# swyoon/Diffusion-by-MaxEntIRL

Hardware: AMD Instinct MI355X
Metric: images/sec (CIFAR-10 DDPM T=10 generation) (higher is better)
Workload: dtype bf16; 1 GPU; CIFAR-10 DDPM U-Net (35.7M params) VARSampler T=10 generation, 256 images/GPU/step, 3x32x32 (BASELINE configs[1]); noise drawn inside the step; global_batch=256, T=10, parallelism=dp1 (independent trajectories, no collective)

## Files before the change

### diffusion-by-maxentirl_amd/csrc/conv_common.h

```cpp
#pragma once
#include "common.h"

struct ConvArgs {
    const bf16* in0;
    const bf16* in1;
    const bf16* w;
    const float* bias;
    const float* addvec;
    const bf16* residual;
    const bf16* mask_src;
    void* out;
    int N, IH, IW, C0, C1, OH, OW, Cout;
    int ksize, stride, pad, ups, act, addvec_ld, in_mode, out_mode;
    int P, pre_act;
    int TWl, THl, SUBS;
    int HH, HWd;
    int PT, CT, CB, KST;
    int tile_px;
    int lds_buf;
    float mask_slope;
    int stagger;
    int RP, SP;
    float* gn_stats;
    bf16* gn_out;
    const float* gn_gamma;
    const float* gn_beta;
    float gn_eps;
    int gn_flags;
    int res_is_mask;
    int xcd_order;
};

__device__ __forceinline__ int dxmi_xcd_logical(int b, int G, int on) {
    if (!on) return b;
    const int x = b & 7, k = b >> 3;
    const int q = G >> 3, r = G & 7;
    return x * q + (x < r ? x : r) + k;
}

__device__ __forceinline__ float dxmi_row16_sum(float t) {
#define DXMI_DPP_ADD(ctrl) t += __builtin_bit_cast(float, __builtin_amdgcn_update_dpp(0, __builtin_bit_cast(int, t), ctrl, 0xf, 0xf, false))
    DXMI_DPP_ADD(0xB1);
    DXMI_DPP_ADD(0x4E);
    DXMI_DPP_ADD(0x141);
    DXMI_DPP_ADD(0x140);
#undef DXMI_DPP_ADD
    return t;
}

__device__ __forceinline__ void dxmi_stats4(const bf16x4& o, float (&st)[4]) {
    const bf16x2 lo = {o[0], o[1]}, hi = {o[2], o[3]};
    const bf16x2 one = {(bf16)1.f, (bf16)1.f};
    st[0] = __builtin_amdgcn_fdot2_f32_bf16(lo, one, st[0], false);
    st[1] = __builtin_amdgcn_fdot2_f32_bf16(lo, lo, st[1], false);
    st[2] = __builtin_amdgcn_fdot2_f32_bf16(hi, one, st[2], false);
    st[3] = __builtin_amdgcn_fdot2_f32_bf16(hi, hi, st[3], false);
}

__device__ __forceinline__ bool conv_block_to_tile(const ConvArgs& p, int bid, int& pt, int& cot) {
    const int xcd = bid & 7;
    const int j = bid >> 3;
    pt = (j / p.CT) * 8 + xcd;
    cot = j % p.CT;
    return pt < p.PT;
}

template <int MB, int NB, bool WIDE>
__device__ __forceinline__ void conv_epilogue(const ConvArgs& p, f32x16 (&acc)[MB][NB], int pt, int n0, int oy0,
                                              int ox0, int pxblk0, int cb0, int lane) {
    const bool rows = p.in_mode == DXMI_IN_ROWS_F32;
    const int TW = 1 << p.TWl, TH = 1 << p.THl;
    const int h = lane >> 5;
    const bool vec_ok = WIDE || ((p.out_mode != DXMI_OUT_NCHW_F32) && ((p.Cout & 3) == 0));
#pragma unroll
    for (int nb = 0; nb < NB; ++nb) {
        const int pix = (pxblk0 + nb) * 32 + (lane & 31);
        size_t opix;
        int n = 0, oy = 0, ox = 0;
        bool pvalid;
        if (rows) {
            const long grow = (long)pt * p.tile_px + pix;
            pvalid = grow < p.P;
            opix = (size_t)grow;
        } else {
            const int x = pix & (TW - 1);
            const int y = (pix >> p.TWl) & (TH - 1);
            const int sub = pix >> (p.TWl + p.THl);
            n = n0 + sub; oy = oy0 + y; ox = ox0 + x;
            pvalid = n < p.N;
            opix = ((size_t)n * p.OH + oy) * p.OW + ox;
        }
#pragma unroll
        for (int mb = 0; mb < MB; ++mb) {
#pragma unroll
            for (int g = 0; g < 4; ++g) {
                const int co = (cb0 + mb) * 32 + 8 * g + 4 * h;
                float v[4];
#pragma unroll
                for (int e = 0; e < 4; ++e) v[e] = acc[mb][nb][4 * g + e];
                if (pvalid && co < p.Cout) {
                    if (vec_ok) {
                        if (p.bias) {
                            const f32x4 bv = *reinterpret_cast<const f32x4*>(p.bias + co);
#pragma unroll
                            for (int e = 0; e < 4; ++e) v[e] += bv[e];
                        }
                        if (p.addvec) {
                            const f32x4 av = *reinterpret_cast<const f32x4*>(p.addvec + (size_t)n * p.addvec_ld + co);
#pragma unroll
                            for (int e = 0; e < 4; ++e) v[e] += av[e];
                        }
                        if (p.residual) {
                            const bf16x4 rv = *reinterpret_cast<const bf16x4*>(p.residual + opix * p.Cout + co);
#pragma unroll
                            for (int e = 0; e < 4; ++e) v[e] += (float)rv[e];
                        }
                        if (p.mask_src) {
                            const bf16x4 mv = *reinterpret_cast<const bf16x4*>(p.mask_src + opix * p.Cout + co);
#pragma unroll
                            for (int e = 0; e < 4; ++e) v[e] *= ((float)mv[e] > 0.f ? 1.f : p.mask_slope);
                        }
#pragma unroll
                        for (int e = 0; e < 4; ++e) v[e] = dxmi_act(v[e], p.act);
                        if (p.out_mode == DXMI_OUT_ROWS_F32) {
                            f32x4 o;
#pragma unroll
                            for (int e = 0; e < 4; ++e) o[e] = v[e];
                            *reinterpret_cast<f32x4*>(reinterpret_cast<float*>(p.out) + opix * p.Cout + co) = o;
                        } else {
                            bf16x4 o;
#pragma unroll
                            for (int e = 0; e < 4; ++e) o[e] = (bf16)v[e];
                            *reinterpret_cast<bf16x4*>(reinterpret_cast<bf16*>(p.out) + opix * p.Cout + co) = o;
                        }
                    } else if constexpr (!WIDE) {
#pragma unroll
                        for (int e = 0; e < 4; ++e) {
                            if (co + e < p.Cout) {
                                float r = v[e] + (p.bias ? p.bias[co + e] : 0.f);
                                if (p.addvec) r += p.addvec[(size_t)n * p.addvec_ld + co + e];
                                r = dxmi_act(r, p.act);
                                if (p.out_mode == DXMI_OUT_NCHW_F32)
                                    reinterpret_cast<float*>(p.out)[(((size_t)n * p.Cout + co + e) * p.OH + oy) * p.OW + ox] = r;
                                else if (p.out_mode == DXMI_OUT_ROWS_F32)
                                    reinterpret_cast<float*>(p.out)[opix * p.Cout + co + e] = r;
                                else
                                    reinterpret_cast<bf16*>(p.out)[opix * p.Cout + co + e] = (bf16)r;
                            }
                        }
                    }
                }
            }
        }
    }
}

enum class ConvKernel { igemm, pipe, stream1x1, stem, ws, ws8, sm, rw, rw8, head };

struct ConvPlan {
    ConvKernel kind;
    int t0, t1, t2;
    ConvArgs args;
    int grid;
    size_t lds;
    int id;
    int stats_tile;
    bool gn_out;
};

bool conv_ws_select(const ConvArgs& a, ConvPlan* p);
bool conv_ws8_select(const ConvArgs& a, ConvPlan* p);
bool conv_sm_select(const ConvArgs& a, ConvPlan* p);
bool conv1x1_rw_select(const ConvArgs& a, ConvPlan* p);
bool conv1x1_rw8_select(const ConvArgs& a, ConvPlan* p);
bool conv_head_select(const ConvArgs& a, ConvPlan* p);
bool conv_stem_select(const ConvArgs& a, ConvPlan* p);
bool conv_pipe_select(const ConvArgs& a, ConvPlan* p);
int conv_ws_launch(const ConvPlan& p, hipStream_t st);
int conv_ws8_launch(const ConvPlan& p, hipStream_t st);
int conv_sm_launch(const ConvPlan& p, hipStream_t st);
int conv1x1_rw_launch(const ConvPlan& p, hipStream_t st);
int conv1x1_rw8_launch(const ConvPlan& p, hipStream_t st);
int conv_head_launch(const ConvPlan& p, hipStream_t st);
int conv_stem_launch(const ConvPlan& p, hipStream_t st);
int conv_pipe_launch(const ConvPlan& p, hipStream_t st);

template <typename T>
bool conv_zero_page(const void*& page, const T& symbol) {
    void* zp = nullptr;
    if (!page && hipGetSymbolAddress(&zp, symbol) == hipSuccess) page = zp;
    return page != nullptr;
}

int conv_plan(const dxmi_conv_desc* d, ConvPlan* p);
```

### diffusion-by-maxentirl_amd/csrc/conv_ws.hip

```cpp
#include "conv_common.h"
#include <stdlib.h>
#include <type_traits>


#ifdef DXMI_CONV_STAMPS
__device__ unsigned g_ws_wait[256][176];
extern "C" int dxmi_debug_read_ws_stamps(void* dst, int bytes) {
    return (int)hipMemcpyFromSymbol(dst, HIP_SYMBOL(g_ws_wait), bytes, 0, hipMemcpyDeviceToHost);
}
#define WS_STAMPED_BARRIER(idx)                                                                     \
    do {                                                                                            \
        const unsigned long long t0_ = __builtin_amdgcn_s_memtime();                                \
        ws_barrier();                                                                               \
        const unsigned long long t1_ = __builtin_amdgcn_s_memtime();                                \
        if (wave == 0 && lane == 0 && (idx) < 160 && blockIdx.x < 256) g_ws_wait[blockIdx.x][(idx)] = (unsigned)(t1_ - t0_); \
    } while (0)
#define WS_CLOCKSTAMP(slot, cond)                                                                    \
    do {                                                                                            \
        if ((cond) && lane == 0 && blockIdx.x < 256) {                                              \
            g_ws_wait[blockIdx.x][(slot)] = (unsigned)__builtin_amdgcn_s_memtime();                 \
            g_ws_wait[blockIdx.x][(slot) + 1] = (unsigned)__builtin_amdgcn_s_memrealtime();         \
        }                                                                                           \
    } while (0)
#define WS_TSTAMP(slot, cond)                                                                        \
    do {                                                                                            \
        if ((cond) && lane == 0 && blockIdx.x < 256) g_ws_wait[blockIdx.x][(slot)] = (unsigned)__builtin_amdgcn_s_memtime(); \
    } while (0)
#define WS_DBG(bit) (p.stagger & (bit))
#else
#define WS_STAMPED_BARRIER(idx) ws_barrier()
#define WS_TSTAMP(slot, cond) do {} while (0)
#define WS_CLOCKSTAMP(slot, cond) do {} while (0)
#define WS_DBG(bit) 0
#endif

__device__ unsigned long long g_ws_clock[4];
extern "C" int dxmi_conv_ws_last_clock(unsigned long long* host_out4) {
    return hipMemcpyFromSymbol(host_out4, HIP_SYMBOL(g_ws_clock), 4 * sizeof(unsigned long long), 0, hipMemcpyDeviceToHost) == hipSuccess ? DXMI_OK
                                                                                                                                          : DXMI_ELAUNCH;
}

namespace {

constexpr int WS_A_SLOT = 8192;
constexpr int WS_RING = 6;
constexpr int WS_A_RING = WS_RING * WS_A_SLOT;
constexpr int WS_RO = 256 * 256;
constexpr int WS_TB = 1024;
constexpr int WS_HALO_BLOCKS = 22;
constexpr int WS_HALO = WS_HALO_BLOCKS * 1024;

__device__ uint4 ws_zero16 = {0u, 0u, 0u, 0u};

#define WS_GPTR(p) ((const __attribute__((address_space(1))) void*)(p))
#define WS_LPTR(p) ((__attribute__((address_space(3))) void*)(p))

__device__ __forceinline__ void ws_barrier() { asm volatile("s_waitcnt lgkmcnt(0)\n\ts_barrier" ::: "memory"); }

#define WS_INTERLEAVE_4()                                       \
    do {                                                        \
        _Pragma("unroll") for (int i_ = 0; i_ < 4; ++i_) {      \
            __builtin_amdgcn_sched_group_barrier(0x008, 3, 0);  \
            __builtin_amdgcn_sched_group_barrier(0x100, 1, 0);  \
        }                                                       \
        __builtin_amdgcn_sched_group_barrier(0x008, 4, 0);      \
    } while (0)
#define WS_INTERLEAVE_8()                                       \
    do {                                                        \
        _Pragma("unroll") for (int i_ = 0; i_ < 8; ++i_) {      \
            __builtin_amdgcn_sched_group_barrier(0x008, 1, 0);  \
            __builtin_amdgcn_sched_group_barrier(0x100, 1, 0);  \
        }                                                       \
        __builtin_amdgcn_sched_group_barrier(0x008, 8, 0);      \
    } while (0)

__device__ __forceinline__ void ws_wait_vm(int n) {
    switch (n >> 1) {
    case 0: asm volatile("s_waitcnt vmcnt(0)" ::: "memory"); break;
    case 1: asm volatile("s_waitcnt vmcnt(2)" ::: "memory"); break;
    case 2: asm volatile("s_waitcnt vmcnt(4)" ::: "memory"); break;
    case 3: asm volatile("s_waitcnt vmcnt(6)" ::: "memory"); break;
    case 4: asm volatile("s_waitcnt vmcnt(8)" ::: "memory"); break;
    case 5: asm volatile("s_waitcnt vmcnt(10)" ::: "memory"); break;
    case 6: asm volatile("s_waitcnt vmcnt(12)" ::: "memory"); break;
    case 7: asm volatile("s_waitcnt vmcnt(14)" ::: "memory"); break;
    case 8: asm volatile("s_waitcnt vmcnt(16)" ::: "memory"); break;
    case 9: asm volatile("s_waitcnt vmcnt(18)" ::: "memory"); break;
    case 10: asm volatile("s_waitcnt vmcnt(20)" ::: "memory"); break;
    default: asm volatile("s_waitcnt vmcnt(22)" ::: "memory"); break;
    }
}

struct WsTile {
    int cot, n0, oy0, ox0;
};

#ifdef WS_VALU_PIECES
typedef float ws_f32x2 __attribute__((ext_vector_type(2)));
struct WsValuLoad {
    u32x4 r[2];
    ws_f32x2 A[4], B[4];
    unsigned sink;
    __device__ __forceinline__ void init(int lane) {
        for (int k = 0; k < 2; ++k) r[k] = u32x4{0x3f803f00u + lane + k, 0xbf803e80u + k, 0x3e003f80u + lane, 0x40003f00u - k};
        for (int i = 0; i < 4; ++i) {
            A[i] = ws_f32x2{0.9f + 0.01f * lane, 1.1f - 0.01f * i};
            B[i] = ws_f32x2{0.05f * i, -0.03f * lane};
        }
        sink = 0;
    }
    __device__ __forceinline__ void run() {
#pragma unroll
        for (int k = 0; k < WS_VALU_PIECES; ++k) {
            u32x4& raw = r[k & 1];
#pragma unroll
            for (int i = 0; i < 4; ++i) {
                ws_f32x2 x = {__builtin_bit_cast(float, raw[i] << 16), __builtin_bit_cast(float, raw[i] & 0xffff0000u)};
                ws_f32x2 y = x * A[i] + B[i];
                const ws_f32x2 t = y * ws_f32x2{-1.4426950408889634f, -1.4426950408889634f};
                ws_f32x2 e = {__builtin_amdgcn_exp2f(t[0]), __builtin_amdgcn_exp2f(t[1])};
                e = e + ws_f32x2{1.f, 1.f};
                const ws_f32x2 rc = {__builtin_amdgcn_rcpf(e[0]), __builtin_amdgcn_rcpf(e[1])};
                y = y * rc;
                bf16x2 o = {(bf16)y[0], (bf16)y[1]};
                sink ^= __builtin_bit_cast(unsigned, o);
            }
            raw += u32x4{0x10001u, 0x20003u, 0x10002u, 0x30001u};
        }
    }
};
#define WS_VALU_DECL(lane_) WsValuLoad vl_; vl_.init(lane_)
#define WS_VALU_RUN() vl_.run()
#define WS_VALU_DONE() do { if (vl_.sink == 0x12345u) reinterpret_cast<volatile unsigned*>(p.out)[0] = vl_.sink; } while (0)
#else
#define WS_VALU_DECL(lane_) do {} while (0)
#define WS_VALU_RUN() do {} while (0)
#define WS_VALU_DONE() do {} while (0)
#endif

template <int TW>
__device__ __forceinline__ void conv_ws_body(const ConvArgs& p) {
    constexpr int TH = 256 / TW, HP = TW == 32 ? 34 : 18, HH = TH + 2, TWl = TW == 32 ? 5 : 4;
    extern __shared__ __attribute__((aligned(1024))) char smem[];
    char* const halo0 = smem;
    char* const aring = smem + 2 * WS_HALO;
    char* const ro = aring + WS_A_RING;
    float* const tb = reinterpret_cast<float*>(ro + WS_RO);

    const int tid = threadIdx.x, lane = tid & 63;
    const int wave = __builtin_amdgcn_readfirstlane(tid >> 6);
    const int txn = p.OW / TW, tyn = p.OH / TH;
    const int nchunks = (p.C0 + p.C1) / 32;
    const int S = 9 * nchunks;
    const int ntiles = p.PT * p.CT;
    const int ups = p.ups ? 1 : 0;

    auto tile_of = [&](int q, WsTile& t) {
        t.cot = q % p.CT;
        const int pt = q / p.CT;
        const int tx = pt % txn, ty = (pt / txn) % tyn;
        t.n0 = pt / (txn * tyn);
        t.oy0 = ty * TH;
        t.ox0 = tx * TW;
    };

    const int q0 = dxmi_xcd_logical(blockIdx.x, gridDim.x, p.xcd_order);
    int q = q0;
    if (q >= ntiles) return;
    const int qstride = gridDim.x;
    if (blockIdx.x == 0 && tid == 0) {
        g_ws_clock[0] = __builtin_amdgcn_s_memtime();
        g_ws_clock[1] = __builtin_amdgcn_s_memrealtime();
    }
    WS_CLOCKSTAMP(172, wave == 0);

    if (wave < 4) {
        const int ch = wave & 1, ph = wave >> 1;
        const int px = lane & 15, kg = lane >> 4;
        constexpr int BROW = TW == 32 ? 2 : 1;
        int bbase[3];
#pragma unroll
        for (int kx = 0; kx < 3; ++kx)
            bbase[kx] = ((ph * (8 / BROW) * HP + px + kx) * 64) + ((kg ^ (2 * (((px + kx) >> 2) & 1))) << 4);
        const char* const abase = aring + ch * 2048 + ((kg >> 1) * 4096) + ((px + 32 * (kg & 1)) << 4);
        f32x4 acc[4][8];
#pragma unroll
        for (int cb = 0; cb < 4; ++cb)
#pragma unroll
            for (int nb = 0; nb < 8; ++nb)
#pragma unroll
                for (int r = 0; r < 4; ++r) acc[cb][nb][r] = 0.f;
        bf16x8 A0[4], A1[4], Bx[4], By[4];
        auto read_a = [&](int u, bf16x8 (&A)[4]) {
            const char* as = abase + (u % WS_RING) * WS_A_SLOT;
#pragma unroll
            for (int cb = 0; cb < 4; ++cb) A[cb] = *reinterpret_cast<const bf16x8*>(as + (cb >> 1) * 1024 + (cb & 1) * 256);
        };
        auto read_b = [&](int u, int half, bf16x8 (&B)[4]) {
            const int t = u % 9, ky = t / 3, kx = t % 3;
            const char* hb = halo0 + ((u / 9) & 1) * WS_HALO + bbase[kx];
#pragma unroll
            for (int i = 0; i < 4; ++i) {
                const int nb = half * 4 + i;
                B[i] = *reinterpret_cast<const bf16x8*>(hb + ((nb / BROW + ky) * HP + (nb % BROW) * 16) * 64);
            }
        };
        auto mfma16 = [&](const bf16x8 (&A)[4], const bf16x8 (&B)[4], int half) {
#pragma unroll
            for (int i = 0; i < 4; ++i)
#pragma unroll
                for (int cb = 0; cb < 4; ++cb)
                    acc[cb][half * 4 + i] = __builtin_amdgcn_mfma_f32_16x16x32_bf16(A[cb], B[i], acc[cb][half * 4 + i], 0, 0, 0);
        };
        const float slope = dxmi_act_slope(p.act);
        const bool has_res = p.residual != nullptr;

        ws_barrier();
        WS_CLOCKSTAMP(168, wave == 0);
        read_a(0, A0);
        read_b(0, 0, Bx);
        int stamp_i = 0;
        (void)stamp_i;
        for (;;) {
            const bool more = q + qstride < ntiles;
            for (int c = 0; c < nchunks; c += 2) {
#pragma unroll
                for (int u = 0; u < 18; ++u) {
                    read_b(u, 1, By);
                    if (u & 1) mfma16(A1, Bx, 0); else mfma16(A0, Bx, 0);
                    WS_INTERLEAVE_4();
                    if (u % 3 == 2) { if (!(WS_DBG(16))) WS_STAMPED_BARRIER(stamp_i + c * 9 + u); }
                    if (u & 1) read_a(u + 1, A0); else read_a(u + 1, A1);
                    read_b(u + 1, 0, Bx);
                    if (u & 1) mfma16(A1, By, 1); else mfma16(A0, By, 1);
                    WS_INTERLEAVE_8();
                    __builtin_amdgcn_sched_barrier(0);
                }
            }
            WS_TSTAMP(158, wave == 0 && q == q0);
            ws_barrier();
            WS_TSTAMP(159, wave == 0 && q == q0);
            {
                const bool plain = p.act == DXMI_ACT_NONE;
                char* const rowb = ro + ((ph * 128 + px) << 8) + 8 * (kg & 1);
                const bool want_stats = p.gn_stats != nullptr;
                const int cot_ = q % p.CT;
                float* const stp = want_stats ? p.gn_stats + ((size_t)((q / p.CT) * 2 + ph) * (p.Cout >> 1) + cot_ * 64 + ch * 32 + kg * 2) * 2 : nullptr;
                auto epi = [&](auto RES, auto MASK, auto ACT, auto STATS) {
                    constexpr bool kRes = decltype(RES)::value, kMask = decltype(MASK)::value, kAct = decltype(ACT)::value, kStats = decltype(STATS)::value;
#pragma unroll
                    for (int cb = 0; cb < 4; ++cb) {
                        float st[4] = {0.f, 0.f, 0.f, 0.f};
                        const int co = ch * 64 + cb * 16 + 4 * kg;
                        const f32x4 b0 = *reinterpret_cast<const f32x4*>(tb + co), t0 = *reinterpret_cast<const f32x4*>(tb + 128 + co);
                        f32x4 bv;
#pragma unroll
                        for (int e = 0; e < 4; ++e) bv[e] = b0[e] + t0[e];
                        char* const a0 = rowb + (((ch * 8 + cb * 2 + (kg >> 1)) ^ px) << 4);
                        bf16x4 r[8];
                        if constexpr (kRes) {
#pragma unroll
                            for (int nb = 0; nb < 8; ++nb) r[nb] = *reinterpret_cast<const bf16x4*>(a0 + nb * 4096);
                        }
#pragma unroll
                        for (int nb = 0; nb < 8; ++nb) {
                            f32x4 v;
#pragma unroll
                            for (int e = 0; e < 4; ++e) v[e] = acc[cb][nb][e] + bv[e];
                            if constexpr (kRes) {
                                if constexpr (kMask) {
#pragma unroll
                                    for (int e = 0; e < 4; ++e) v[e] *= ((float)r[nb][e] > 0.f ? 1.f : p.mask_slope);
                                } else {
#pragma unroll
                                    for (int e = 0; e < 4; ++e) v[e] += (float)r[nb][e];
                                }
                            }
                            if constexpr (kAct) {
#pragma unroll
                                for (int e = 0; e < 4; ++e) v[e] = dxmi_act_lin(v[e], slope);
                            }
                            bf16x4 o;
#pragma unroll
                            for (int e = 0; e < 4; ++e) o[e] = (bf16)v[e];
                            *reinterpret_cast<bf16x4*>(a0 + nb * 4096) = o;
                            if constexpr (kStats) dxmi_stats4(o, st);
#pragma unroll
                            for (int e = 0; e < 4; ++e) acc[cb][nb][e] = 0.f;
                        }
                        if constexpr (kStats) {
#pragma unroll
                            for (int e = 0; e < 4; ++e) st[e] = dxmi_row16_sum(st[e]);
                            if (px == 0 && cot_ * 128 + co < p.Cout) {
                                f32x4 sv;
#pragma unroll
                                for (int e = 0; e < 4; ++e) sv[e] = st[e];
                                *reinterpret_cast<f32x4*>(stp + cb * 16) = sv;
                            }
                        }
                    }
                };
                using T_ = std::true_type;
                using F_ = std::false_type;
                const bool is_mask = has_res && p.res_is_mask;
                if (plain && !is_mask) {
                    if (has_res) { if (want_stats) epi(T_{}, F_{}, F_{}, T_{}); else epi(T_{}, F_{}, F_{}, F_{}); }
                    else { if (want_stats) epi(F_{}, F_{}, F_{}, T_{}); else epi(F_{}, F_{}, F_{}, F_{}); }
                } else if (!want_stats) {
                    if (is_mask) { if (plain) epi(T_{}, T_{}, F_{}, F_{}); else epi(T_{}, T_{}, T_{}, F_{}); }
                    else if (has_res) epi(T_{}, F_{}, T_{}, F_{});
                    else epi(F_{}, F_{}, T_{}, F_{});
                } else {
                    if (is_mask) epi(T_{}, T_{}, T_{}, T_{});
                    else if (has_res) epi(T_{}, F_{}, T_{}, T_{});
                    else epi(F_{}, F_{}, T_{}, T_{});
                }
            }
            WS_TSTAMP(166, wave == 0 && q == q0);
            ws_barrier();
            WS_TSTAMP(157, wave == 0 && q == q0);
            if (!more) {
                WS_CLOCKSTAMP(170, wave == 0);
                break;
            }
            q += qstride;
            stamp_i += S;
        }
    } else if (wave < 6) {
        WS_VALU_DECL(lane);
        const int lw = wave - 4;
        const char* const wb = reinterpret_cast<const char*>(p.w) + (size_t)lane * 16;
        WsTile cur;
        tile_of(q, cur);
        auto issue_tap = [&](int cot, int g) {
            if (WS_DBG(1)) return;
            const int c = g / 9, t = g - c * 9;
            char* dst = aring + (g % WS_RING) * WS_A_SLOT + lw * 4096;
            const char* src = wb + ((size_t)(t * p.KST + c * 2 + lw) * p.CB) * 1024;
#pragma unroll
            for (int f = 0; f < 4; ++f) {
                const int cb = cot * 4 + f < p.CB ? cot * 4 + f : p.CB - 1;
                __builtin_amdgcn_global_load_lds(WS_GPTR(src + (size_t)cb * 1024), WS_LPTR(dst + f * 1024), 16, 0, 0);
            }
        };
        u32x4 fq[2][3][4];
        auto load_tap = [&](int cot, int g, u32x4 (&f)[4]) {
            const int c = g / 9, t = g - c * 9;
            const char* src = wb + ((size_t)(t * p.KST + c * 2 + lw) * p.CB) * 1024;
#pragma unroll
            for (int k = 0; k < 4; ++k) {
                const int cb = cot * 4 + k < p.CB ? cot * 4 + k : p.CB - 1;
                asm volatile("global_load_dwordx4 %0, %1, off" : "=v"(f[k]) : "v"(src + (size_t)cb * 1024) : "memory");
            }
        };
        auto store_tap = [&](int g, const u32x4 (&f)[4]) {
            char* dst = aring + (g % WS_RING) * WS_A_SLOT + lw * 4096 + lane * 16;
#pragma unroll
            for (int k = 0; k < 4; ++k) *reinterpret_cast<u32x4*>(dst + k * 1024) = f[k];
        };
        const int NG = S / 3;
        auto load_group = [&](int G, int cot_cur, int cot_nxt, u32x4 (&f)[3][4]) {
            const bool nx = G >= NG;
            const int g0 = (nx ? G - NG : G) * 3, cot = nx ? cot_nxt : cot_cur;
#pragma unroll
            for (int j = 0; j < 3; ++j) load_tap(cot, g0 + j, f[j]);
        };
        auto store_group = [&](int G, const u32x4 (&f)[3][4]) {
#pragma unroll
            for (int j = 0; j < 3; ++j) store_tap((G & 1) * 3 + j, f[j]);
        };
        if (WS_DBG(1)) {}
        const int t2l = lw * 64 + lane, prl = t2l >> 4;
        const int lpar_l0 = prl * p.Cout + (((t2l & 15) ^ prl) * 8), lpar_l1 = prl * p.Cout + (((t2l & 15) ^ (prl | 8)) * 8);
        const int c8e_l = (t2l & 15) ^ prl, c8o_l = (t2l & 15) ^ (prl | 8);
        const int kpc_l = (32 + nchunks - 2) / (nchunks - 1);
        const char* const zero_page_l = reinterpret_cast<const char*>(p.mask_src);
        bool first_tile_l = true, first_group0 = true;
        load_group(0, cur.cot, cur.cot, fq[0]);
        load_group(1, cur.cot, cur.cot, fq[1]);
        asm volatile("s_waitcnt vmcnt(12)" ::: "memory");
        store_group(0, fq[0]);
        asm volatile("s_waitcnt lgkmcnt(0)" ::: "memory");
        load_group(2, cur.cot, cur.cot, fq[0]);
        ws_barrier();
        bool first_tile = true;
        for (;;) {
            const bool more = q + qstride < ntiles;
            WsTile nxt = cur;
            if (more) tile_of(q + qstride, nxt);
            if (!first_tile && lw == 0 && !(WS_DBG(8))) {
                const int co_a = cur.cot * 128 + lane, co_b = co_a + 64 < p.Cout ? co_a + 64 : p.Cout - 1;
                if (p.bias) {
                    __builtin_amdgcn_global_load_lds(WS_GPTR(p.bias + co_a), WS_LPTR(tb), 4, 0, 0);
                    __builtin_amdgcn_global_load_lds(WS_GPTR(p.bias + co_b), WS_LPTR(tb + 64), 4, 0, 0);
                }
                if (p.addvec) {
                    const float* av = p.addvec + (size_t)cur.n0 * p.addvec_ld;
                    __builtin_amdgcn_global_load_lds(WS_GPTR(av + co_a), WS_LPTR(tb + 128), 4, 0, 0);
                    __builtin_amdgcn_global_load_lds(WS_GPTR(av + co_b), WS_LPTR(tb + 192), 4, 0, 0);
                }
            }
            const bf16* const res_t = p.residual + ((((size_t)cur.n0 * p.OH + cur.oy0) * p.OW + cur.ox0) * p.Cout + cur.cot * 128);
            const bool res_here = !first_tile_l && p.residual != nullptr && !(WS_DBG(8));
            first_tile_l = false;
            first_tile = false;
            for (int G0 = 0; G0 < NG; G0 += 2) {
#pragma unroll
                for (int j = 0; j < 2; ++j) {
                    const int G = G0 + j;
                    if (G > 0 || first_group0) {
                        asm volatile("s_waitcnt vmcnt(12)" ::: "memory");
                        store_group(G + 1, fq[(j + 1) & 1]);
                        asm volatile("s_waitcnt lgkmcnt(0)" ::: "memory");
                    }
                    if (res_here && G > 0) {
                        const int cg = (G - 1) / 3, g3 = (G - 1) - cg * 3;
                        if (cg + 1 < nchunks) {
                            const int k0 = cg * kpc_l < 32 ? cg * kpc_l : 32, k1 = k0 + kpc_l < 32 ? k0 + kpc_l : 32;
                            const int i0 = g3 < 2 ? 3 * g3 : 6, i1 = g3 < 2 ? 3 * g3 + 3 : 12;
                            const int ka = k0 + i0 < k1 ? k0 + i0 : k1, kb = k0 + i1 < k1 ? k0 + i1 : k1;
#pragma unroll 1
                            for (int k = ka; k < kb; ++k) {
                                const int rel = ((k >> (TWl - 3)) * p.OW + (k & (TW / 8 - 1)) * 8) * p.Cout + ((k & 1) ? lpar_l1 : lpar_l0);
                                const bool ok = cur.cot * 128 + ((k & 1) ? c8o_l : c8e_l) * 8 < p.Cout;
                                const void* g = ok ? (const void*)(res_t + rel) : (const void*)zero_page_l;
                                __builtin_amdgcn_global_load_lds(WS_GPTR(g), WS_LPTR(ro + (k * 128 + lw * 64) * 16), 16, 0, 0);
                            }
                        }
                    }
                    if (G > 0 || first_group0) load_group(G + 3, cur.cot, more ? nxt.cot : cur.cot, fq[(j + 1) & 1]);
                    WS_TSTAMP(151, wave == 4 && G == 0 && q == q0 + qstride);
                    WS_VALU_RUN();
                    if (!(WS_DBG(16))) ws_barrier();
                }
            }
            first_group0 = false;
            if (more) {
                asm volatile("s_waitcnt vmcnt(12)" ::: "memory");
                store_group(1, fq[1]);
                asm volatile("s_waitcnt lgkmcnt(0)" ::: "memory");
                load_group(3, nxt.cot, nxt.cot, fq[1]);
            }
            ws_barrier();
            ws_barrier();
            WS_TSTAMP(150, wave == 4 && q == q0);
            if (!more) break;
            q += qstride;
            cur = nxt;
        }
        asm volatile("s_waitcnt vmcnt(0)" ::: "memory");
        WS_VALU_DONE();
    } else if (wave == 6) {
        WS_VALU_DECL(lane);
        constexpr int HBA = WS_HALO_BLOCKS;
        const char* const zero_page = reinterpret_cast<const char*>(p.mask_src);
        int hrel0[HBA], hrel1[HBA];
        unsigned m_in = 0, m_top = 0, m_bot = 0, m_left = 0, m_right = 0;
#pragma unroll
        for (int k = 0; k < HBA; ++k) {
            const int hp = k * 16 + (lane >> 2);
            const int hy = hp / HP, hx = hp - hy * HP;
            const int rel = ((hy - 1) >> ups) * p.IW + ((hx - 1) >> ups);
            const int j8 = ((lane & 3) ^ (2 * ((hx >> 2) & 1))) * 8;
            hrel0[k] = (rel * p.C0 + j8) * 2;
            hrel1[k] = (rel * p.C1 + j8) * 2;
            m_in |= (unsigned)(hy < HH && hx < TW + 2) << k;
            m_top |= (unsigned)(hy == 0) << k;
            m_bot |= (unsigned)(hy == HH - 1) << k;
            m_left |= (unsigned)(hx == 0) << k;
            m_right |= (unsigned)(hx == TW + 1) << k;
        }
        unsigned hmask = 0;
        int hbase0 = 0, hbase1 = 0;
        auto halo_plan = [&](const WsTile& t) {
            hmask = m_in;
            if (t.oy0 == 0) hmask &= ~m_top;
            if (t.oy0 + TH == p.OH) hmask &= ~m_bot;
            if (t.ox0 == 0) hmask &= ~m_left;
            if (t.ox0 + TW == p.OW) hmask &= ~m_right;
            const int pix = (t.n0 * p.IH + (t.oy0 >> ups)) * p.IW + (t.ox0 >> ups);
            hbase0 = pix * p.C0 * 2;
            hbase1 = pix * p.C1 * 2;
        };
        auto halo_issue = [&](int c, char* buf, int ka, int kb) {
            if (WS_DBG(2)) return;
            const int cbase = c * 32;
            const bool first = cbase < p.C0;
            const char* base = reinterpret_cast<const char*>(first ? p.in0 : p.in1) + (first ? cbase : cbase - p.C0) * 2 + (first ? hbase0 : hbase1);
#pragma unroll
            for (int k = 0; k < HBA; ++k) {
                if (k < ka || k >= kb) continue;
                const char* g = (hmask >> k) & 1 ? base + (first ? hrel0[k] : hrel1[k]) : zero_page;
                __builtin_amdgcn_global_load_lds(WS_GPTR(g), WS_LPTR(buf + k * 1024), 16, 0, 0);
            }
        };
        WsTile cur;
        tile_of(q, cur);
        if (!p.bias) { tb[lane] = 0.f; tb[64 + lane] = 0.f; }
        if (!p.addvec) { tb[128 + lane] = 0.f; tb[192 + lane] = 0.f; }
        halo_plan(cur);
        halo_issue(0, halo0, 0, HBA);
        if (!(WS_DBG(8))) {
            const int co_a = cur.cot * 128 + lane, co_b = co_a + 64 < p.Cout ? co_a + 64 : p.Cout - 1;
            if (p.bias) {
                __builtin_amdgcn_global_load_lds(WS_GPTR(p.bias + co_a), WS_LPTR(tb), 4, 0, 0);
                __builtin_amdgcn_global_load_lds(WS_GPTR(p.bias + co_b), WS_LPTR(tb + 64), 4, 0, 0);
            }
            if (p.addvec) {
                const float* av = p.addvec + (size_t)cur.n0 * p.addvec_ld;
                __builtin_amdgcn_global_load_lds(WS_GPTR(av + co_a), WS_LPTR(tb + 128), 4, 0, 0);
                __builtin_amdgcn_global_load_lds(WS_GPTR(av + co_b), WS_LPTR(tb + 192), 4, 0, 0);
            }
        }
        asm volatile("s_waitcnt vmcnt(0)" ::: "memory");
        ws_barrier();
        WsTile nxt = cur;
        for (;;) {
            const bool more = q + qstride < ntiles;
            for (int c = 0; c < nchunks; ++c) {
                const bool wrap = c + 1 == nchunks;
                if (wrap && more) {
                    tile_of(q + qstride, nxt);
                    halo_plan(nxt);
                }
                const bool do_halo = !wrap || more;
                char* const hbuf = halo0 + ((c + 1) & 1) * WS_HALO;
                const int hc = wrap ? 0 : c + 1;
#pragma unroll
                for (int t = 0; t < 9; ++t) {
                    if (t < 8 && do_halo) halo_issue(hc, hbuf, 3 * t, 3 * t + 3 < HBA ? 3 * t + 3 : HBA);
                    if (t == 8) asm volatile("s_waitcnt vmcnt(0)" ::: "memory");
                    if (t % 3 == 2) { WS_VALU_RUN(); if (!(WS_DBG(16))) ws_barrier(); }
                }
            }
            ws_barrier();
            ws_barrier();
            if (!more) break;
            q += qstride;
            cur = nxt;
        }
        WS_VALU_DONE();
    } else if (wave == 7) {
        WS_VALU_DECL(lane);
        const char* const zero_page = reinterpret_cast<const char*>(p.mask_src);
        const int prA = lane >> 4, prB = 4 + (lane >> 4), lc = lane & 15;
        const int lparA[2] = {prA * p.Cout + ((lc ^ prA) * 8), prA * p.Cout + ((lc ^ (prA | 8)) * 8)};
        const int lparB[2] = {prB * p.Cout + ((lc ^ prB) * 8), prB * p.Cout + ((lc ^ (prB | 8)) * 8)};
        const int c8A[2] = {lc ^ prA, lc ^ (prA | 8)}, c8B[2] = {lc ^ prB, lc ^ (prB | 8)};
        auto tile_base = [&](const WsTile& t) -> size_t {
            return (((size_t)t.n0 * p.OH + t.oy0) * p.OW + t.ox0) * p.Cout + t.cot * 128;
        };
        auto piece_u = [&](int k) -> int { return ((k >> (TWl - 3)) * p.OW + (k & (TW / 8 - 1)) * 8) * p.Cout; };
        WsTile cur;
        tile_of(q, cur);
        if (p.residual != nullptr && !(WS_DBG(8))) {
            const bf16* rb = p.residual + tile_base(cur);
#pragma unroll 1
            for (int k = 0; k < 32; ++k) {
                const int u = piece_u(k);
                const void* ga = cur.cot * 128 + c8A[k & 1] * 8 < p.Cout ? (const void*)(rb + u + lparA[k & 1]) : (const void*)zero_page;
                const void* gb = cur.cot * 128 + c8B[k & 1] * 8 < p.Cout ? (const void*)(rb + u + lparB[k & 1]) : (const void*)zero_page;
                __builtin_amdgcn_global_load_lds(WS_GPTR(ga), WS_LPTR(ro + (k * 128) * 16), 16, 0, 0);
                __builtin_amdgcn_global_load_lds(WS_GPTR(gb), WS_LPTR(ro + (k * 128 + 64) * 16), 16, 0, 0);
            }
        }
        ws_barrier();
        bool have_prev = false;
        WsTile prev = cur;
        const int kpc = (32 + nchunks - 2) / (nchunks - 1);
        auto piece_range = [&](int c, int t, int& ka, int& kb) {
            ka = kb = 32;
            if (!have_prev || c + 1 >= nchunks) return;
            const int k0 = c * kpc < 32 ? c * kpc : 32, k1 = k0 + kpc < 32 ? k0 + kpc : 32;
            const int i0 = t < 6 ? t : 6 + 2 * (t - 6), i1 = t < 6 ? t + 1 : i0 + 2;
            ka = k0 + i0 < k1 ? k0 + i0 : k1;
            kb = k0 + i1 < k1 ? k0 + i1 : k1;
        };
        const bool do_drain = !(WS_DBG(4));
        bf16* out_prev = reinterpret_cast<bf16*>(p.out);
        for (;;) {
            const bool more = q + qstride < ntiles;
            WsTile nxt = cur;
            if (more) tile_of(q + qstride, nxt);
            for (int c = 0; c < nchunks; ++c) {
#pragma unroll
                for (int t = 0; t < 9; ++t) {
                    int ka, kb;
                    piece_range(c, t, ka, kb);
                    if (ka < kb && do_drain) {
                        bf16x8 va[2], vb[2];
#pragma unroll
                        for (int u = 0; u < 2; ++u)
                            if (ka + u < kb) {
                                va[u] = *reinterpret_cast<const bf16x8*>(ro + ((ka + u) * 128 + lane) * 16);
                                vb[u] = *reinterpret_cast<const bf16x8*>(ro + ((ka + u) * 128 + 64 + lane) * 16);
                            }
#pragma unroll
                        for (int u = 0; u < 2; ++u)
                            if (ka + u < kb) {
                                const int k = ka + u, pu = piece_u(k);
                                if (prev.cot * 128 + c8A[k & 1] * 8 < p.Cout) *reinterpret_cast<bf16x8*>(out_prev + pu + lparA[k & 1]) = va[u];
                                if (prev.cot * 128 + c8B[k & 1] * 8 < p.Cout) *reinterpret_cast<bf16x8*>(out_prev + pu + lparB[k & 1]) = vb[u];
                            }
                    }
                    asm volatile("s_waitcnt lgkmcnt(0)" ::: "memory");
                    if (t % 3 == 2) { WS_VALU_RUN(); if (!(WS_DBG(16))) ws_barrier(); }
                }
            }
            if (!have_prev) asm volatile("s_waitcnt vmcnt(0)" ::: "memory");
            ws_barrier();
            ws_barrier();
            out_prev = reinterpret_cast<bf16*>(p.out) + tile_base(cur);
            prev = cur;
            have_prev = true;
            if (!more) break;
            q += qstride;
            cur = nxt;
        }
        WS_VALU_DONE();
    }

    {
        const int qlast = q0 + ((ntiles - 1 - q0) / qstride) * qstride;
        WsTile lt;
        tile_of(qlast, lt);
        bf16* const ob = reinterpret_cast<bf16*>(p.out) + ((((size_t)lt.n0 * p.OH + lt.oy0) * p.OW + lt.ox0) * p.Cout + lt.cot * 128);
        const int t2 = tid & 127, kq = tid >> 7;
        const int pr = t2 >> 4;
#pragma unroll
        for (int i = 0; i < 8; i += 4) {
            bf16x8 v[4];
#pragma unroll
            for (int u = 0; u < 4; ++u) v[u] = *reinterpret_cast<const bf16x8*>(ro + (((i + u) * 4 + kq) * 128 + t2) * 16);
#pragma unroll
            for (int u = 0; u < 4; ++u) {
                const int k = (i + u) * 4 + kq;
                const int lp = k * 8 + pr;
                const int c8 = (t2 & 15) ^ (lp & 15);
                const int rel = ((lp >> TWl) * p.OW + (lp & (TW - 1))) * p.Cout + c8 * 8;
                if (lt.cot * 128 + c8 * 8 < p.Cout) *reinterpret_cast<bf16x8*>(ob + rel) = v[u];
            }
        }
        WS_CLOCKSTAMP(174, wave == 0);
    }
    if (blockIdx.x == 0 && tid == 0) {
        g_ws_clock[2] = __builtin_amdgcn_s_memtime();
        g_ws_clock[3] = __builtin_amdgcn_s_memrealtime();
    }
}

template <int TW>
__global__ __launch_bounds__(512, 1) void conv_ws_kernel(ConvArgs p) {
    conv_ws_body<TW>(p);
}

}

bool conv_ws_select(const ConvArgs& a, ConvPlan* p) {
    if (a.in_mode != DXMI_IN_NHWC_BF16 || a.out_mode != DXMI_OUT_NHWC_BF16) return false;
    if (a.ksize != 3 || a.stride != 1 || a.pad != 1 || a.ups == 2 || (a.mask_src && a.residual) || a.act == DXMI_ACT_SILU) return false;
    if (a.Cout % 64 != 0 || (a.C0 + a.C1) % 32 != 0 || a.C0 % 32 != 0) return false;
    const int TW = a.OW >= 32 ? 32 : a.OW;
    if (TW != 32 && TW != 16) return false;
    const int TH = 256 / TW;
    if (a.OH % TH != 0 || a.OW % TW != 0) return false;
    const int nchunks = (a.C0 + a.C1) / 32;
    if ((9 * nchunks) % WS_RING != 0 || nchunks % 2 != 0) return false;
    if (nchunks < 4) return false;
    const int min_tiles = dxmi_tuning("conv_ws_min_tiles");
    if ((long)a.N * (a.OH / TH) * (a.OW / TW) * ((a.Cout + 127) / 128) < min_tiles) return false;
    if ((long)a.N * a.IH * a.IW * (a.C0 > a.C1 ? a.C0 : a.C1) * 2 >= (1L << 31)) return false;
    ConvArgs& b = p->args;
    if (a.mask_src) { b.residual = a.mask_src; b.res_is_mask = 1; }
    b.SUBS = 1;
    b.PT = a.N * (a.OH / TH) * (a.OW / TW);
    b.CT = (a.Cout + 127) / 128;
    b.tile_px = 256;
    b.xcd_order = 1;
    b.stagger = 0;
    p->kind = ConvKernel::ws; p->t0 = TW;
    p->grid = b.PT * b.CT < 256 ? b.PT * b.CT : 256;
    p->lds = 2 * WS_HALO + WS_A_RING + WS_RO + WS_TB;
    p->id = 400000 + TW;
    p->stats_tile = 128;
    return true;
}

int conv_ws_launch(const ConvPlan& p, hipStream_t st) {
    static const void* zero_page = nullptr;
    DXMI_CHECK_ARG(conv_zero_page(zero_page, HIP_SYMBOL(ws_zero16)), "dxmi_conv2d_fwd(ws): hipGetSymbolAddress(ws_zero16) failed");
    ConvArgs b = p.args;
    b.mask_src = reinterpret_cast<const bf16*>(zero_page);
#ifdef DXMI_CONV_STAMPS
    static const int dbg = getenv("DXMI_CONV_WS_DBG") ? atoi(getenv("DXMI_CONV_WS_DBG")) : 0;
    b.stagger = dbg;
#endif
    static bool attr_set = false;
    if (!attr_set) {
        (void)hipFuncSetAttribute(reinterpret_cast<const void*>(conv_ws_kernel<32>), hipFuncAttributeMaxDynamicSharedMemorySize, 160 * 1024);
        (void)hipFuncSetAttribute(reinterpret_cast<const void*>(conv_ws_kernel<16>), hipFuncAttributeMaxDynamicSharedMemorySize, 160 * 1024);
        attr_set = true;
    }
    if (p.t0 == 32) hipLaunchKernelGGL(conv_ws_kernel<32>, dim3(p.grid), dim3(512), p.lds, st, b);
    else hipLaunchKernelGGL(conv_ws_kernel<16>, dim3(p.grid), dim3(512), p.lds, st, b);
    DXMI_CHECK_LAUNCH("dxmi_conv2d_fwd(ws)");
    return DXMI_OK;
}
```

Measured before the change: 6920 images/s.

## Add specialized warp-specialized conv kernel for nearest-upsample 3x3 convolutions

Adds a dedicated warp-specialized kernel for 3x3 convs that follow a 2x nearest upsample. It reads the low-resolution input directly and reuses each input column for two output columns by combining horizontal tap partial sums with DPP lane shifts. The aim is to remove redundant loads and MFMA work on duplicated upsampled pixels, with separate producer, compute and store waves. It only applies to 16/32-wide outputs with channel counts divisible by 64, and it adds a large amount of hand-tuned layout and synchronisation code that could go wrong.

```diff
diff --git a/diffusion-by-maxentirl_amd/csrc/conv_common.h b/diffusion-by-maxentirl_amd/csrc/conv_common.h
--- a/diffusion-by-maxentirl_amd/csrc/conv_common.h
+++ b/diffusion-by-maxentirl_amd/csrc/conv_common.h
@@ -169,6 +169,7 @@
 };
 
 bool conv_ws_select(const ConvArgs& a, ConvPlan* p);
+bool conv_ws_up_select(const ConvArgs& a, ConvPlan* p);
 bool conv_ws8_select(const ConvArgs& a, ConvPlan* p);
 bool conv_sm_select(const ConvArgs& a, ConvPlan* p);
 bool conv1x1_rw_select(const ConvArgs& a, ConvPlan* p);
@@ -177,6 +178,7 @@
 bool conv_stem_select(const ConvArgs& a, ConvPlan* p);
 bool conv_pipe_select(const ConvArgs& a, ConvPlan* p);
 int conv_ws_launch(const ConvPlan& p, hipStream_t st);
+int conv_ws_up_launch(const ConvPlan& p, hipStream_t st);
 int conv_ws8_launch(const ConvPlan& p, hipStream_t st);
 int conv_sm_launch(const ConvPlan& p, hipStream_t st);
 int conv1x1_rw_launch(const ConvPlan& p, hipStream_t st);
diff --git a/diffusion-by-maxentirl_amd/csrc/conv_ws.hip b/diffusion-by-maxentirl_amd/csrc/conv_ws.hip
--- a/diffusion-by-maxentirl_amd/csrc/conv_ws.hip
+++ b/diffusion-by-maxentirl_amd/csrc/conv_ws.hip
@@ -683,10 +683,12 @@
     p->lds = 2 * WS_HALO + WS_A_RING + WS_RO + WS_TB;
     p->id = 400000 + TW;
     p->stats_tile = 128;
+    conv_ws_up_select(a, p);
     return true;
 }
 
 int conv_ws_launch(const ConvPlan& p, hipStream_t st) {
+    if (p.t1 == 1) return conv_ws_up_launch(p, st);
     static const void* zero_page = nullptr;
     DXMI_CHECK_ARG(conv_zero_page(zero_page, HIP_SYMBOL(ws_zero16)), "dxmi_conv2d_fwd(ws): hipGetSymbolAddress(ws_zero16) failed");
     ConvArgs b = p.args;
diff --git a/diffusion-by-maxentirl_amd/csrc/conv_ws_up.hip b/diffusion-by-maxentirl_amd/csrc/conv_ws_up.hip
--- /dev/null
+++ b/diffusion-by-maxentirl_amd/csrc/conv_ws_up.hip
@@ -0,0 +1,300 @@
+#include "conv_common.h"
+#include <type_traits>
+
+namespace {
+
+constexpr int UP_A_CHUNK = 9 * 4096;
+constexpr int UP_HALO = 6 * 1024;
+constexpr int UP_RO = 256 * 128;
+constexpr int UP_LDS = 2 * UP_A_CHUNK + 2 * UP_HALO + UP_RO;
+
+__device__ __forceinline__ void up_barrier() { asm volatile("s_waitcnt lgkmcnt(0)\n\ts_barrier" ::: "memory"); }
+
+struct UpTile {
+    int cot, pt, n0, oy0;
+};
+
+template <int TW>
+__global__ __launch_bounds__(512, 1) void conv_ws_up_kernel(ConvArgs p) {
+    constexpr int IW = TW / 2, TH = 256 / TW, ROWB = IW * 64;
+    constexpr int NF = TW == 32 ? 6 : 9;
+    extern __shared__ __attribute__((aligned(1024))) char smem[];
+    char* const abuf = smem;
+    char* const hbuf = smem + 2 * UP_A_CHUNK;
+    char* const ro = hbuf + 2 * UP_HALO;
+
+    const int tid = threadIdx.x, lane = tid & 63;
+    const int wave = __builtin_amdgcn_readfirstlane(tid >> 6);
+    const int tyn = p.OH / TH;
+    const int nchunks = p.C0 / 32;
+    const int ntiles = p.PT * p.CT;
+    auto tile_of = [&](int q, UpTile& t) {
+        t.cot = q % p.CT;
+        t.pt = q / p.CT;
+        t.n0 = t.pt / tyn;
+        t.oy0 = (t.pt % tyn) * TH;
+    };
+    const int q0 = dxmi_xcd_logical(blockIdx.x, gridDim.x, p.xcd_order);
+    int q = q0;
+    if (q >= ntiles) return;
+    const int qstride = gridDim.x;
+    const int px = lane & 15, kg = lane >> 4;
+
+    if (wave < 4) {
+        const int w = wave;
+        auto Yl = [](int j) { return TW == 32 ? j : (j >> 1) * 4 + (j & 1); };
+        const char* const bbase = hbuf + px * 64 + ((kg ^ (2 * ((px >> 2) & 1))) << 4);
+        const char* const abase = abuf + (kg >> 1) * 2048 + (w >> 1) * 1024 + ((px + 32 * (kg & 1) + 16 * (w & 1)) << 4);
+        f32x4 acc[3][8];
+#pragma unroll
+        for (int b = 0; b < 3; ++b)
+#pragma unroll
+            for (int j = 0; j < 8; ++j)
+#pragma unroll
+                for (int e = 0; e < 4; ++e) acc[b][j][e] = 0.f;
+        bf16x8 A[2], Bf[2][NF];
+        auto read_a = [&](int P, int t, bf16x8& a) { a = *reinterpret_cast<const bf16x8*>(abase + P * UP_A_CHUNK + t * 4096); };
+        auto read_b = [&](int P, bf16x8 (&B)[NF]) {
+#pragma unroll
+            for (int h = 0; h < NF; ++h) B[h] = *reinterpret_cast<const bf16x8*>(bbase + P * UP_HALO + h * ROWB);
+        };
+        const float slope = dxmi_act_slope(p.act);
+        const bool has_res = p.residual != nullptr, is_mask = has_res && p.res_is_mask, want_stats = p.gn_stats != nullptr;
+        const int lanepix = TW == 32 ? 2 * px : (px >> 3) * 32 + 2 * (px & 7);
+        char* const rob = ro + lanepix * 128 + (((w * 2 + (kg >> 1)) ^ (px & 7)) << 4) + (kg & 1) * 8;
+
+        up_barrier();
+        read_b(0, Bf[0]);
+        read_a(0, 0, A[0]);
+        for (;;) {
+            const bool more = q + qstride < ntiles;
+            UpTile cur;
+            tile_of(q, cur);
+            for (int c = 0; c < nchunks; c += 2) {
+#pragma unroll
+                for (int u = 0; u < 18; ++u) {
+                    const int P = u / 9, t = u % 9, a = t / 3, b = t % 3;
+                    if (t < 8) {
+                        read_a(P, t + 1, A[(u + 1) & 1]);
+                    } else {
+                        up_barrier();
+                        read_b(P ^ 1, Bf[P ^ 1]);
+                        read_a(P ^ 1, 0, A[(u + 1) & 1]);
+                    }
+#pragma unroll
+                    for (int j = 0; j < 8; ++j)
+                        acc[b][j] = __builtin_amdgcn_mfma_f32_16x16x32_bf16(A[u & 1], Bf[P][(Yl(j) + a + 1) >> 1], acc[b][j], 0, 0, 0);
+                    __builtin_amdgcn_sched_barrier(0);
+                }
+            }
+            {
+                const int co = cur.cot * 64 + w * 16 + 4 * kg;
+                f32x4 bv = {0.f, 0.f, 0.f, 0.f};
+                if (p.bias) bv = *reinterpret_cast<const f32x4*>(p.bias + co);
+                if (p.addvec) {
+                    const f32x4 av = *reinterpret_cast<const f32x4*>(p.addvec + (size_t)cur.n0 * p.addvec_ld + co);
+#pragma unroll
+                    for (int e = 0; e < 4; ++e) bv[e] += av[e];
+                }
+                const size_t tile_px = ((size_t)cur.n0 * p.OH + cur.oy0) * TW;
+                float* const stp = want_stats ? p.gn_stats + (size_t)cur.pt * 2 * p.Cout + co : nullptr;
+                auto epi = [&](auto RES, auto MASK, auto STATS) {
+                    constexpr bool kRes = decltype(RES)::value, kMask = decltype(MASK)::value, kStats = decltype(STATS)::value;
+                    bf16x4 r[8][2];
+                    if constexpr (kRes) {
+                        const bf16* const rp = p.residual + (tile_px + lanepix) * p.Cout + co;
+#pragma unroll
+                        for (int j = 0; j < 8; ++j)
+#pragma unroll
+                            for (int x = 0; x < 2; ++x) r[j][x] = *reinterpret_cast<const bf16x4*>(rp + (size_t)(Yl(j) * TW + x) * p.Cout);
+                    }
+                    float st[4] = {0.f, 0.f, 0.f, 0.f};
+#pragma unroll
+                    for (int j = 0; j < 8; ++j) {
+                        f32x4 v[2];
+#pragma unroll
+                        for (int e = 0; e < 4; ++e) {
+                            float r0s, r2s;
+                            asm volatile("s_nop 1\n\tv_mov_b32_dpp %0, %1 row_shr:1 row_mask:0xf bank_mask:0xf bound_ctrl:1" : "=v"(r0s) : "v"(acc[0][j][e]));
+                            asm volatile("s_nop 1\n\tv_mov_b32_dpp %0, %1 row_shl:1 row_mask:0xf bank_mask:0xf bound_ctrl:1" : "=v"(r2s) : "v"(acc[2][j][e]));
+                            if (TW == 16) {
+                                r0s = (px & 7) == 0 ? 0.f : r0s;
+                                r2s = (px & 7) == 7 ? 0.f : r2s;
+                            }
+                            v[0][e] = (r0s + acc[1][j][e]) + acc[2][j][e];
+                            v[1][e] = (acc[0][j][e] + acc[1][j][e]) + r2s;
+                        }
+#pragma unroll
+                        for (int x = 0; x < 2; ++x) {
+#pragma unroll
+                            for (int e = 0; e < 4; ++e) v[x][e] += bv[e];
+                            if constexpr (kRes) {
+                                if constexpr (kMask) {
+#pragma unroll
+                                    for (int e = 0; e < 4; ++e) v[x][e] *= ((float)r[j][x][e] > 0.f ? 1.f : p.mask_slope);
+                                } else {
+#pragma unroll
+                                    for (int e = 0; e < 4; ++e) v[x][e] += (float)r[j][x][e];
+                                }
+                            }
+                            bf16x4 o;
+#pragma unroll
+                            for (int e = 0; e < 4; ++e) o[e] = (bf16)dxmi_act_lin(v[x][e], slope);
+                            *reinterpret_cast<bf16x4*>(rob + (Yl(j) * TW + x) * 128) = o;
+                            if constexpr (kStats) dxmi_stats4(o, st);
+                        }
+#pragma unroll
+                        for (int b = 0; b < 3; ++b)
+#pragma unroll
+                            for (int e = 0; e < 4; ++e) acc[b][j][e] = 0.f;
+                        if constexpr (kStats) {
+                            if (j == 3 || j == 7) {
+                                f32x4 sv;
+#pragma unroll
+                                for (int e = 0; e < 4; ++e) { sv[e] = dxmi_row16_sum(st[e]); st[e] = 0.f; }
+                                if (px == 0) *reinterpret_cast<f32x4*>(stp + (size_t)(j >> 2) * p.Cout) = sv;
+                            }
+                        }
+                    }
+                };
+                using T_ = std::true_type;
+                using F_ = std::false_type;
+                if (is_mask) { if (want_stats) epi(T_{}, T_{}, T_{}); else epi(T_{}, T_{}, F_{}); }
+                else if (has_res) { if (want_stats) epi(T_{}, F_{}, T_{}); else epi(T_{}, F_{}, F_{}); }
+                else { if (want_stats) epi(F_{}, F_{}, T_{}); else epi(F_{}, F_{}, F_{}); }
+            }
+            up_barrier();
+            if (!more) break;
+            q += qstride;
+        }
+    } else if (wave < 7) {
+        const int lw = wave - 4;
+        const char* const wb = reinterpret_cast<const char*>(p.w) + (size_t)lane * 16;
+        const int p16 = lane >> 2, j8 = ((lane & 3) ^ (2 * ((p16 >> 2) & 1))) * 8;
+        int hrow[2], hcol;
+#pragma unroll
+        for (int m = 0; m < 2; ++m) hrow[m] = TW == 32 ? lw * 2 + m : (lw * 2 + m) * 2 + (p16 >> 3);
+        hcol = TW == 32 ? p16 : p16 & 7;
+        int fq = q, fc = 0;
+        u32x4 fw[12], fh[2];
+        bool hok[2];
+        auto fetch = [&]() {
+            UpTile t;
+            tile_of(fq, t);
+            const char* src = wb + ((size_t)(fc * 2) * p.CB + t.cot * 2) * 1024;
+#pragma unroll
+            for (int m = 0; m < 12; ++m) {
+                const int tap = lw * 3 + (m >> 2), ks = (m >> 1) & 1, cbl = m & 1;
+                fw[m] = *reinterpret_cast<const u32x4*>(src + ((size_t)(tap * p.KST + ks) * p.CB + cbl) * 1024);
+            }
+#pragma unroll
+            for (int m = 0; m < 2; ++m) {
+                const int r = (t.oy0 >> 1) - 1 + hrow[m];
+                hok[m] = r >= 0 && r < p.IH;
+                const int rc = r < 0 ? 0 : (r < p.IH ? r : p.IH - 1);
+                fh[m] = *reinterpret_cast<const u32x4*>(p.in0 + (((size_t)t.n0 * p.IH + rc) * IW + hcol) * p.C0 + fc * 32 + j8);
+            }
+            if (++fc == nchunks) {
+                fc = 0;
+                if (fq + qstride < ntiles) fq += qstride;
+            }
+        };
+        auto store = [&](int P) {
+            char* const da = abuf + P * UP_A_CHUNK + (lw * 12) * 1024 + lane * 16;
+#pragma unroll
+            for (int m = 0; m < 12; ++m) *reinterpret_cast<u32x4*>(da + m * 1024) = fw[m];
+            char* const dh = hbuf + P * UP_HALO + (lw * 2) * 1024 + lane * 16;
+#pragma unroll
+            for (int m = 0; m < 2; ++m) *reinterpret_cast<u32x4*>(dh + m * 1024) = hok[m] ? fh[m] : u32x4{0u, 0u, 0u, 0u};
+        };
+        fetch();
+        store(0);
+        fetch();
+        up_barrier();
+        for (;;) {
+            const bool more = q + qstride < ntiles;
+            for (int c = 0; c < nchunks; c += 2) {
+#pragma unroll
+                for (int P = 0; P < 2; ++P) {
+                    store(P ^ 1);
+                    asm volatile("s_waitcnt lgkmcnt(0)" ::: "memory");
+                    fetch();
+                    up_barrier();
+                }
+            }
+            up_barrier();
+            if (!more) break;
+            q += qstride;
+        }
+    } else {
+        const int dpx = lane >> 3, dsl = lane & 7;
+        const int nchunks_d = nchunks - 1;
+        const int kpc = (32 + nchunks_d - 1) / nchunks_d;
+        bool have_prev = false;
+        bf16* out_prev = reinterpret_cast<bf16*>(p.out);
+        for (int i = 0;; ++i) {
+            const bool more = q + qstride < ntiles;
+            if (i == 0) up_barrier();
+            for (int c = 0; c < nchunks; ++c) {
+                if (have_prev) {
+                    const int ka = c * kpc < 32 ? c * kpc : 32, kb = ka + kpc < 32 ? ka + kpc : 32;
+#pragma unroll 2
+                    for (int k = ka; k < kb; ++k) {
+                        const int pix = k * 8 + dpx;
+                        const bf16x8 v = *reinterpret_cast<const bf16x8*>(ro + (k * 64 + lane) * 16);
+                        *reinterpret_cast<bf16x8*>(out_prev + (size_t)pix * p.Cout + (dsl ^ ((pix >> 1) & 7)) * 8) = v;
+                    }
+                }
+                up_barrier();
+            }
+            up_barrier();
+            UpTile cur;
+            tile_of(q, cur);
+            out_prev = reinterpret_cast<bf16*>(p.out) + (((size_t)cur.n0 * p.OH + cur.oy0) * TW) * p.Cout + cur.cot * 64;
+            have_prev = true;
+            if (!more) break;
+            q += qstride;
+        }
+    }
+
+    {
+        UpTile lt;
+        tile_of(q0 + ((ntiles - 1 - q0) / qstride) * qstride, lt);
+        bf16* const ob = reinterpret_cast<bf16*>(p.out) + (((size_t)lt.n0 * p.OH + lt.oy0) * TW) * p.Cout + lt.cot * 64;
+        bf16x8 v[4];
+#pragma unroll
+        for (int u = 0; u < 4; ++u) v[u] = *reinterpret_cast<const bf16x8*>(ro + ((wave * 4 + u) * 64 + lane) * 16);
+#pragma unroll
+        for (int u = 0; u < 4; ++u) {
+            const int pix = (wave * 4 + u) * 8 + (lane >> 3);
+            *reinterpret_cast<bf16x8*>(ob + (size_t)pix * p.Cout + ((lane & 7) ^ ((pix >> 1) & 7)) * 8) = v[u];
+        }
+    }
+}
+
+}
+
+bool conv_ws_up_select(const ConvArgs& a, ConvPlan* p) {
+    if (a.ups != 1 || a.C1 != 0 || a.OW != 2 * a.IW || a.OH != 2 * a.IH || (a.OW != 32 && a.OW != 16)) return false;
+    if (a.Cout % 64 != 0 || a.C0 % 64 != 0 || a.C0 < 128 || a.OH % (256 / a.OW) != 0) return false;
+    ConvArgs& b = p->args;
+    b.PT = a.N * (a.OH / (256 / a.OW));
+    b.CT = a.Cout / 64;
+    p->t1 = 1;
+    p->grid = b.PT * b.CT < 256 ? b.PT * b.CT : 256;
+    p->lds = UP_LDS;
+    return true;
+}
+
+int conv_ws_up_launch(const ConvPlan& p, hipStream_t st) {
+    static bool attr_set = false;
+    if (!attr_set) {
+        (void)hipFuncSetAttribute(reinterpret_cast<const void*>(conv_ws_up_kernel<32>), hipFuncAttributeMaxDynamicSharedMemorySize, 160 * 1024);
+        (void)hipFuncSetAttribute(reinterpret_cast<const void*>(conv_ws_up_kernel<16>), hipFuncAttributeMaxDynamicSharedMemorySize, 160 * 1024);
+        attr_set = true;
+    }
+    if (p.t0 == 32) hipLaunchKernelGGL(conv_ws_up_kernel<32>, dim3(p.grid), dim3(512), p.lds, st, p.args);
+    else hipLaunchKernelGGL(conv_ws_up_kernel<16>, dim3(p.grid), dim3(512), p.lds, st, p.args);
+    DXMI_CHECK_LAUNCH("dxmi_conv2d_fwd(ws up)");
+    return DXMI_OK;
+}
```

New measurement: 7053 images/s, median of 6. +1.9%, better.
